# EavianWoo/SinGS

Measured on AMD Instinct MI355X. Metric: rendered views/sec fwd+bwd, 200k Gaussians @1080p, higher is better.
Workload: dtype f32; 1 GPU; S(200000,1920,1080,deg=3,seed=3): 200000 Gaussians, 1920x1080, SH deg 3, fwd+bwd, R=780064 (tile,Gaussian) pairs, every view of a step within 0.1 % of that (cameras a few cm apart), frame-parallel dp1; gaussians=200000, width=1920, height=1080, sh_degree=3, num_rendered=780064, tile_list_max=135, frames_per_launch=8, streams=2, regularisers=False, forward_only=False, hip_graph=False, reduction=fold of 2 gradient row(s) for 16 views + collective in 1 chunk(s), gradient_rows=2, parallelism=dp1

## Files before the change

sings_amd/csrc/sg_binning.hip:

```cpp
#include "sg_sort.h"
#include <atomic>

#define SG_SCAN_NQ 6
__device__ __forceinline__ void sg_scan_derive(uint32_t v, uint32_t q[SG_SCAN_NQ])
{
    const uint32_t seg = sg_nseg(v);
    q[0] = v; q[1] = seg ? seg : 1u; q[2] = seg; q[3] = v > SG_WSORT_MAX ? 1u : 0u; q[4] = sg_group_slots(v);
    q[5] = (v > SG_WSORT_MAX / 2 ? 1u : 0u) | (v > SG_TILE_ROW_LONG / 2 ? 1u << 20 : 0u);
}

__device__ __forceinline__ void sg_publish_count(unsigned long long *signal, uint32_t R, uint32_t flags)
{
    if (signal) __hip_atomic_store(signal, (1ull << 63) | ((unsigned long long)flags << 32) | R, __ATOMIC_RELEASE, __HIP_MEMORY_SCOPE_SYSTEM);
}

template <int SG_SCAN_BS>
__global__ void __launch_bounds__(SG_SCAN_BS)
sg_tile_scan_kernel(int T, int gx, int tpt, const uint32_t *__restrict__ tile_count,
                    uint2 *__restrict__ ranges, uint32_t *__restrict__ cursor, uint32_t *__restrict__ header,
                    uint32_t cap, uint32_t sort_cap, uint32_t rank_cap, uint4 *__restrict__ plan,
                    uint32_t *__restrict__ ck_start, uint32_t items_cap, int short_lists, unsigned long long *signal, size_t bin_stride,
                    int direct)
{
    constexpr int NQ = SG_SCAN_NQ;
    __shared__ uint32_t wsum[NQ][SG_SCAN_BS / 64];
    __shared__ uint32_t carry[NQ];
    {
        const size_t off = (size_t)blockIdx.y * bin_stride;
        tile_count = sg_at(tile_count, off); ranges = sg_at(ranges, off); cursor = sg_at(cursor, off); header = sg_at(header, off);
        plan = sg_at(plan, off); ck_start = sg_at(ck_start, off);
        if (signal) signal += blockIdx.y;
    }
    const int tid = threadIdx.x, lane = tid & 63, wid = tid >> 6;
    const int first = blockIdx.x * SG_SCAN_BS * tpt;
// ... 518 lines not shown
        if (tid == 0 && L.gslot > g0) atomicAdd(&header[7], L.gslot - g0);
    }
}

__global__ void __launch_bounds__(256)
sg_group_sort_kernel(const uint32_t *__restrict__ header, const uint2 *__restrict__ groups, const uint64_t *__restrict__ pair_keys,
                     const uint64_t *__restrict__ scratch, uint32_t *__restrict__ point_list, uint64_t *__restrict__ point_keys,
                     size_t bin_stride)
{
    __shared__ uint64_t s[SG_WSORT_MAX + SG_RANKSORT_MAX];
    {
        const size_t off = (size_t)blockIdx.y * bin_stride;
        header = sg_at(header, off); groups = sg_at(groups, off); pair_keys = sg_at(pair_keys, off); scratch = sg_at(scratch, off);
        point_list = sg_at(point_list, off); point_keys = sg_at(point_keys, off);
    }
    const int tid = threadIdx.x;
    const uint32_t nslots = header[1] || header[7] == 0u ? 0u : header[6];
    for (uint32_t gi = blockIdx.x; gi < nslots; gi += gridDim.x) {
        const uint2 g = groups[gi];
        const uint32_t len = g.y & 0x7ffu, tile = g.y >> 11;
        if (len == 0u) continue;
        const uint32_t start = g.x & ~SG_GROUP_IN_A;
        const uint64_t *src = ((g.x & SG_GROUP_IN_A) ? pair_keys : scratch) + start;
        __syncthreads();
        sg_sort_short_list(src, (int)len, s, s + SG_WSORT_MAX, tid);
        for (uint32_t i = tid; i < len; i += 256) {
            const uint64_t k = s[i];
            point_list[start + i] = (uint32_t)k;
            if (point_keys) point_keys[start + i] = ((uint64_t)tile << 32) | (k >> 32);
        }
    }
}

static bool sg_dyn_lds_limit(int which, const void *fn, int bytes)
{
    static std::atomic<signed char> state[2][64];
    int dev = 0;
    if (hipGetDevice(&dev) != hipSuccess || dev < 0 || dev >= 64)
        return hipFuncSetAttribute(fn, hipFuncAttributeMaxDynamicSharedMemorySize, bytes) == hipSuccess || ((void)hipGetLastError(), false);
    signed char st = state[which][dev].load(std::memory_order_acquire);
    if (st == 0) {
        st = hipFuncSetAttribute(fn, hipFuncAttributeMaxDynamicSharedMemorySize, bytes) == hipSuccess ? 1 : -1;
        if (st < 0) (void)hipGetLastError();
        state[which][dev].store(st, std::memory_order_release);
    }
    return st > 0;
}

void sg_launch_binning(const SgCam &c, const SgBatch &bt, int P, const int32_t *radii, SgGeom g, SgBin b, size_t cap,
                       int write_keys, hipStream_t st)
{
    (void)radii; (void)P;
    const unsigned K = (unsigned)bt.K;
    const int T = c.gx * c.gy;
    const uint32_t cap32 = sg_cap32(cap);
    uint64_t *pk = write_keys ? b.point_keys : (uint64_t *)nullptr;
    const int short_lists = (c.flags & SG_FLAG_SHORT_LISTS) ? 1 : 0;
    const uint32_t key_pitch = sg_key_pitch(c.gx, c.gy, c.flags);
    const int direct = key_pitch ? 1 : 0;
    bool fused = T <= SG_SS_MAX_TILES && (K == 1 || sg_lds_hist(c.gx, c.gy) || direct);
    if (fused && (size_t)T * 4 + 1024 > 64 * 1024)
        fused = sg_dyn_lds_limit(0, (const void *)sg_scan_scatter_kernel, SG_SS_MAX_TILES * 4);
    if (fused) {
        sg_prof_begin(SG_K_TILE_SCAN, st);
        size_t want = (cap + 4 * SG_SS_THREADS - 1) / (4 * SG_SS_THREADS);
        const int grid = direct ? SG_DIRECT_SCAN_WGS : (int)(want < 8 ? 8 : (want > 256 ? 256 : want));
        hipLaunchKernelGGL(sg_scan_scatter_kernel, dim3(grid, K), dim3(SG_SS_THREADS), (size_t)T * 4, st, T, c.gx, b.tile_count, b.ranges,
                           b.cursor, b.header, cap32, sg_sort_items_cap(T, cap), sg_rank_items_cap(cap), b.plan, b.ck_start,
                           sg_items_cap(T, cap), b.pair_gid, b.pair_tile, b.pair_local, g.depth, b.pair_keys, b.sort_items,
                           b.rank_items, b.items, b.item_w, short_lists, c.count_signal, bt.bin, bt.geom,
                           sg_lds_hist(c.gx, c.gy) ? b.rec_valid : (uint8_t *)nullptr, direct);
        sg_prof_end(SG_K_TILE_SCAN, st);
    } else {
        sg_prof_begin(SG_K_TILE_SCAN, st);
        const int tpt = (T + 65535) / 65536 > 0 ? (T + 65535) / 65536 : 1;
        const int sgrid = (T + 1024 * tpt - 1) / (1024 * tpt) > 0 ? (T + 1024 * tpt - 1) / (1024 * tpt) : 1;
        hipLaunchKernelGGL((sg_tile_scan_kernel<1024>), dim3(sgrid, K), dim3(1024), 0, st, T, c.gx, tpt, b.tile_count, b.ranges, b.cursor,
                           b.header, cap32, sg_sort_items_cap(T, cap), sg_rank_items_cap(cap), b.plan, b.ck_start,
                           sg_items_cap(T, cap), short_lists, c.count_signal, bt.bin, direct);
        sg_prof_end(SG_K_TILE_SCAN, st);
        sg_prof_begin(SG_K_TILE_SCATTER, st);
        size_t want = (((direct || cap < (size_t)T) ? (size_t)T : cap) + 255) / 256;
        int grid = (int)(want < 1 ? 1 : (want > 8192 ? 8192 : want));
        hipLaunchKernelGGL(sg_pair_scatter_kernel, dim3(grid, K), dim3(256), 0, st, b.header, b.pair_gid, b.pair_tile,
                           b.pair_local, g.depth, b.cursor, b.pair_keys, cap32, T, b.plan, b.sort_items, b.rank_items,
                           sg_sort_items_cap(T, cap), sg_rank_items_cap(cap), b.items, sg_items_cap(T, cap), b.item_w, bt.bin, bt.geom,
                           sg_lds_hist(c.gx, c.gy) ? b.rec_valid : (uint8_t *)nullptr, direct);
        sg_prof_end(SG_K_TILE_SCATTER, st);
    }
    if (short_lists) return;
    sg_prof_begin(SG_K_TILE_SORT, st);
    const uint32_t pgrid = sg_sort_items_cap(T, cap) < 512 ? sg_sort_items_cap(T, cap) : 512;
    uint32_t resident = SG_PT_U * SG_PT_THREADS;
    size_t dyn = (size_t)resident * 8 + (size_t)SG_PT_FINE * 4;
    if (!sg_dyn_lds_limit(1, (const void *)sg_tile_partition_kernel, (int)dyn)) { resident = SG_PT_NB; dyn = (size_t)SG_PT_NB * 8; }
    hipLaunchKernelGGL(sg_tile_partition_kernel, dim3(pgrid, K), dim3(SG_PT_THREADS), dyn, st, b.header, b.sort_items,
                       b.pair_keys, b.point_keys, b.rank_items, sg_rank_items_cap(cap), b.point_list, pk,
                       resident > SG_PT_NB ? resident : 0u, bt.bin, b.tile_keys, key_pitch);
    const uint32_t ggrid = sg_rank_items_cap(cap) < 256 ? sg_rank_items_cap(cap) : 256;
    hipLaunchKernelGGL(sg_group_sort_kernel, dim3(ggrid, K), dim3(256), 0, st, b.header, b.rank_items, b.pair_keys, b.point_keys,
                       b.point_list, pk, bt.bin);
    sg_prof_end(SG_K_TILE_SORT, st);
}
```

sings_amd/csrc/sg_host.h:

```cpp
#pragma once
#include "sg_common.h"

#include <math.h>
#include <stdarg.h>
#include <stdio.h>

static inline int sg_failf(const char *fmt, ...)
{
    char msg[256];
    va_list ap;
    va_start(ap, fmt);
    vsnprintf(msg, sizeof msg, fmt, ap);
    va_end(ap);
    return sg_set_error(msg, hipSuccess);
}

static inline int sg_launched(const char *what)
{
    const hipError_t e = hipGetLastError();
    return e == hipSuccess ? 0 : sg_set_error(what, e);
}

static inline void sg_ssim_window(float w[11])
{
    float g[11];
    double s = 0.0;
    for (int x = 0; x < 11; x++) { g[x] = (float)exp(-(double)((x - 5) * (x - 5)) / (2.0 * 1.5 * 1.5)); s += (double)g[x]; }
    for (int x = 0; x < 11; x++) w[x] = g[x] / (float)s;
}

#define SG_CHECK_LAST(what, s, st)                                           \
    do {                                                                     \
        hipError_t e_ = hipGetLastError();                                   \
        if (e_ != hipSuccess) return sg_set_error(what, e_);                 \
        if ((s)->debug) {                                                    \
            e_ = hipStreamSynchronize(st);                                   \
            if (e_ != hipSuccess) return sg_set_error(what, e_);             \
        }                                                                    \
    } while (0)

int sg_launch_linear_bwd_fan(int N, int Cin, int Cout, int act, const float *z, const float *dh, const float *W, float *dz_out,
                             float *dx_out, const SgLinearSide *side, hipStream_t st);
void sg_launch_scales_head(int N, const float *z, float *scales, float *aux, const float *dscales, const float *daux, float *dz,
                           hipStream_t st);
void sg_launch_rows_laplacian(int R, int V, int C, const float *x, const int *row_ptr, const int *col, const float *val,
                              const float *rscale, const int *t_row_ptr, const int *t_row, const float *t_val, void *ws, float *g_ws,
                              float *loss, const float *upstream, float *dL_dx, hipStream_t st);

static inline bool sg_order_applies(const SgCam &c) { return !sg_lds_hist(c.gx, c.gy) && sg_key_pitch_of(false, c.flags) != 0u; }
void sg_launch_preprocess_fwd_ordered(const SgCam &c, const SgBatch &bt, int P, const float *means3D, const float *shs,
                                      const float *colors_precomp, const float *opacities, const float *scales,
                                      const float *rotations, const float *cov3D_precomp, SgGeom g, SgBin b,
                                      size_t cap, int32_t *radii, const uint32_t *order, hipStream_t st);
// ... 2 lines not shown
```

sings_amd/csrc/sg_preprocess.hip:

```cpp
#include "sg_project.h"
#include "sg_host.h"

template <int D, bool NOBIN>
__global__ void __launch_bounds__(256)
sg_preprocess_fwd_kernel(SgCam c, SgBatch bt, int P, const float *__restrict__ means3D,
                         const float *__restrict__ shs, const float *__restrict__ colors_precomp,
                         const float *__restrict__ opacities, const float *__restrict__ scales,
                         const float *__restrict__ rotations, const float *__restrict__ cov3D_precomp,
                         SgGeom g, SgBin bn, uint32_t cap, int32_t *__restrict__ radii, int hist_tiles, int nblocks)
{
    extern __shared__ uint32_t sg_hist_lds[];
    __shared__ uint32_t scratch_all[4][NOBIN ? 1 : 256];
    int gblock, frame;
    if (!sg_block_frame((int)blockIdx.x, bt.K, nblocks, gblock, frame)) return;
    c = sg_frame(c, frame, bt.cam_stride); g = sg_frame(g, (size_t)frame * bt.geom); bn = sg_frame(bn, (size_t)frame * bt.bin);
    radii += (size_t)frame * bt.P;
    const int idx = gblock * 256 + (int)threadIdx.x;
    const int wave = threadIdx.x >> 6;
    const bool live = idx < P;
    constexpr int nc = (D + 1) * (D + 1);
    float sh[nc * 3];
    if (shs && live) {
        const float *src = shs + (size_t)idx * c.M * 3;
        if (D == 3 && c.M == 16) {
// ... 63 lines not shown
    if (P <= 0) return;
    const int nblocks = (P + 255) / 256;
    dim3 grid(sg_frame_grid(nblocks, bt.K)), block(256);
    const int ht = sg_lds_hist(c.gx, c.gy) ? (int)sg_ctr_count((uint32_t)c.gx, (uint32_t)c.gy) : 0;
    const bool ord = order && sg_order_applies(c);
#define SG_PPO(DD, OO) hipLaunchKernelGGL((sg_preprocess_fwd_kernel<DD, OO>), grid, block, (size_t)ht * 4, st, c, bt, P, means3D, shs, \
                                     colors_precomp, opacities, scales, rotations, cov3D_precomp, g, b, sg_cap32(cap), radii, ht, nblocks)
#define SG_PP(DD) do { if (ord) SG_PPO(DD, true); else SG_PPO(DD, false); } while (0)
    int D = colors_precomp ? 0 : c.D;
    sg_prof_begin(SG_K_PREPROCESS_FWD, st);
    switch (D) { case 0: SG_PP(0); break; case 1: SG_PP(1); break; case 2: SG_PP(2); break; default: SG_PP(3); break; }
    if (ord)
        hipLaunchKernelGGL(sg_bin_ordered_kernel, dim3(nblocks, bt.K), block, 0, st, bt, P, g, b, c.gx, sg_key_pitch_of(false, c.flags), order);
    sg_prof_end(SG_K_PREPROCESS_FWD, st);
#undef SG_PP
#undef SG_PPO
}

#define SG_PBWD_PARAMS SgCam c, int P, const float *__restrict__ means3D, const float *__restrict__ shs,                              \
                       const float *__restrict__ colors_precomp, const float *__restrict__ scales,                                \
                       const float *__restrict__ rotations, const float *__restrict__ cov3D_precomp,                              \
                       const int32_t *__restrict__ radii, SgGeom g, SgRec grec,                                                   \
                       size_t cap, const uint32_t *__restrict__ header, const uint8_t *__restrict__ rec_valid, float *__restrict__ dL_dmeans3D, float *__restrict__ dL_dmeans2D, \
                       float *__restrict__ dL_dsh, float *__restrict__ dL_dcolors,                                                \
                       float *__restrict__ dL_dopacity, float *__restrict__ dL_dscales,                                           \
                       float *__restrict__ dL_drots, float *__restrict__ dL_dcov3D
#define SG_PBWD_AUX 0
#include "sg_preprocess_bwd.inc"
#undef SG_PBWD_AUX
#define SG_PBWD_AUX 1
#include "sg_preprocess_bwd.inc"
#undef SG_PBWD_AUX

#define SG_GROW_VEC 4
template <int D>
__global__ void __launch_bounds__(256) __attribute__((amdgpu_waves_per_eu(4, 4)))
sg_gauss_frame_bwd_kernel(SgCam c, SgBatch bt, int P, const float *__restrict__ means3D, const float *__restrict__ shs,
                          const float *__restrict__ scales, const float *__restrict__ rotations,
                          const float *__restrict__ cov3D_precomp, const int32_t *__restrict__ radii, SgGeom g, SgRec grec,
                          size_t cap, const uint32_t *__restrict__ header, const uint8_t *__restrict__ rec_valid,
                          float4 *__restrict__ rows, float *__restrict__ dL_dmeans2D, int nblocks)
{
    __shared__ float lds_all[4][32 * SG_ROW_LDS];
    int gblock, frame;
    if (!sg_block_frame((int)blockIdx.x, bt.K, nblocks, gblock, frame)) return;
    c = sg_frame(c, frame, bt.cam_stride); g = sg_frame(g, (size_t)frame * bt.geom); grec = sg_frame(grec, (size_t)frame * bt.rec);
    header = sg_at(header, (size_t)frame * bt.bin); rec_valid = sg_at(rec_valid, (size_t)frame * bt.bin);
    radii += (size_t)frame * bt.P;
    const int idx = gblock * 256 + (int)threadIdx.x;
    const int lane = threadIdx.x & 63, wave = threadIdx.x >> 6;
    if (idx - lane >= P) return;
    const bool live = idx < P;
    const bool vis = live && radii[idx] > 0 && header[1] == 0u;
    const int Mrows = c.M;
    constexpr int nc = (D + 1) * (D + 1);
    const bool want_sh = shs != nullptr;
    float4 rc = make_float4(0, 0, 0, 0);
    float p[3] = { 0, 0, 0 }, s3[3] = { 0, 0, 0 }, q[4] = { 0, 0, 0, 0 }, sh[nc * 3];
    uint32_t flags = 0;
    if (vis) {
        { const uint2 sl = g.slot[idx]; rc.y = __uint_as_float(sl.x); rc.w = __uint_as_float(sl.y); }
        flags = g.flags[idx];
        p[0] = means3D[3 * idx]; p[1] = means3D[3 * idx + 1]; p[2] = means3D[3 * idx + 2];
        if (!cov3D_precomp) {
            s3[0] = scales[3 * idx]; s3[1] = scales[3 * idx + 1]; s3[2] = scales[3 * idx + 2];
            q[0] = rotations[4 * idx]; q[1] = rotations[4 * idx + 1]; q[2] = rotations[4 * idx + 2]; q[3] = rotations[4 * idx + 3];
        }
    }
    float a9[9];
    sg_sum_records_coop(grec, cap, vis, rc, lane, lds_all[wave], a9, rec_valid);
    if (!live) return;
    float *m2 = dL_dmeans2D + 3 * ((size_t)frame * bt.P + idx);
    if (!vis) { m2[0] = 0.0f; m2[1] = 0.0f; m2[2] = 0.0f; return; }
    SgGaussGrad G;
    sg_project_bwd<D>(c, p, s3, q, cov3D_precomp ? cov3D_precomp + 6 * (size_t)idx : nullptr, nullptr, flags, a9, false, nullptr, G);
    m2[0] = G.g2[0]; m2[1] = G.g2[1]; m2[2] = 0.0f;
    float dRGB[3] = { G.dcol[0], G.dcol[1], G.dcol[2] };
    if (want_sh) {
        int ish = idx;
        asm volatile("" : "+v"(ish), "+v"(G.dmean[2]), "+v"(G.drot[3]));
        const float *src = shs + (size_t)ish * Mrows * 3;
        if (D == 3 && Mrows == 16) {
#pragma unroll
            for (int k = 0; k < nc * 3 / 4; k++) {
                const float4 v = ((const float4 *)src)[k];
                sh[4 * k] = v.x; sh[4 * k + 1] = v.y; sh[4 * k + 2] = v.z; sh[4 * k + 3] = v.w;
            }
        } else {
#pragma unroll
            for (int k = 0; k < nc * 3; k++) sh[k] = src[k];
        }
        float dorig[3] = { p[0] - c.campos[0], p[1] - c.campos[1], p[2] - c.campos[2] };
        float sum2 = dorig[0] * dorig[0] + dorig[1] * dorig[1] + dorig[2] * dorig[2];
        float len = sqrtf(sum2);
        float dir[3] = { dorig[0] / len, dorig[1] / len, dorig[2] / len };
        float db[48];
        sg_sh_basis_grad<D>(dir, db);
#pragma unroll
        for (int ch = 0; ch < 3; ch++) dRGB[ch] = (flags >> ch) & 1u ? 0.0f : G.dcol[ch];
        float ddir[3] = { 0, 0, 0 };
#pragma unroll
        for (int k = 1; k < nc; k++)
#pragma unroll
            for (int ch = 0; ch < 3; ch++) {
                float sv = sh[3 * k + ch] * dRGB[ch];
                ddir[0] += db[3 * k] * sv; ddir[1] += db[3 * k + 1] * sv; ddir[2] += db[3 * k + 2] * sv;
            }
        float inv32 = 1.0f / sqrtf(sum2 * sum2 * sum2);
        float vx = dorig[0], vy = dorig[1], vz = dorig[2];
        G.dmean[0] += ((sum2 - vx * vx) * ddir[0] - vy * vx * ddir[1] - vz * vx * ddir[2]) * inv32;
        G.dmean[1] += (-vx * vy * ddir[0] + (sum2 - vy * vy) * ddir[1] - vz * vy * ddir[2]) * inv32;
        G.dmean[2] += (-vx * vz * ddir[0] - vy * vz * ddir[1] + (sum2 - vz * vz) * ddir[2]) * inv32;
    }
    float4 *o = rows + SG_GROW_VEC * ((size_t)frame * bt.P + idx);
    o[0] = make_float4(G.dmean[0], G.dmean[1], G.dmean[2], G.dop);
    if (cov3D_precomp) {
        o[1] = make_float4(G.g6[0], G.g6[1], G.g6[2], G.g6[3]);
        o[2] = make_float4(G.g6[4], G.g6[5], 0.0f, 0.0f);
    } else {
        o[1] = make_float4(G.dsc[0], G.dsc[1], G.dsc[2], 0.0f);
        o[2] = make_float4(G.drot[0], G.drot[1], G.drot[2], G.drot[3]);
    }
    o[3] = make_float4(dRGB[0], dRGB[1], dRGB[2], 0.0f);
}

template <int D, bool ACC>
__global__ void __launch_bounds__(256) __attribute__((amdgpu_waves_per_eu(4, 4)))
sg_gauss_sum_frames_kernel(SgCam c0, SgBatch bt, int P, const float *__restrict__ means3D, const int32_t *__restrict__ radii0,
                           const uint32_t *__restrict__ header0, const float4 *__restrict__ rows, int g6rows,
                           float *__restrict__ dL_dmeans3D, float *__restrict__ dL_dsh, float *__restrict__ dL_dcolors,
                           float *__restrict__ dL_dopacity, float *__restrict__ dL_dscales, float *__restrict__ dL_drots,
                           float *__restrict__ dL_dcov3D)
{
    __shared__ float lds_all[4][32 * SG_ROW_LDS];
    const int idx = blockIdx.x * blockDim.x + threadIdx.x;
    const int lane = threadIdx.x & 63, wave = threadIdx.x >> 6;
    const int g0 = idx - lane;
    if (g0 >= P) return;
    const bool live = idx < P;
    const int Mrows = c0.M;
    const int nframes = bt.K;
    constexpr int nc = (D + 1) * (D + 1);
    const bool want_sh = dL_dsh != nullptr;
    const bool planar = c0.flags & SG_FLAG_SH_PLANAR;
    const bool staged = D == 3 && Mrows == 16 && want_sh && !planar;
    bool vis_n = live && radii0[idx] > 0 && header0[1] == 0u;
    const float4 z4 = make_float4(0, 0, 0, 0);
    float4 n[SG_GROW_VEC] = { z4, z4, z4, z4 };
    if (vis_n) {
        const float4 *src = rows + SG_GROW_VEC * (size_t)idx;
#pragma unroll
        for (int v = 0; v < SG_GROW_VEC; v++) n[v] = src[v];
    }
    float p[3] = { 0, 0, 0 };
    if (live) { p[0] = means3D[3 * idx]; p[1] = means3D[3 * idx + 1]; p[2] = means3D[3 * idx + 2]; }
    constexpr int NA = 4 * SG_GROW_VEC - 1;
    static_assert(NA * 64 <= 32 * SG_ROW_LDS, "the geometry sums fit the wave's staging block");
    float *sA = lds_all[wave] + lane;
    float A[NA];
#pragma unroll
    for (int k = 0; k < NA; k++) A[k] = 0.0f;
    float acc[nc * 3];
#pragma unroll
    for (int k = 0; k < nc * 3; k++) acc[k] = 0.0f;
    if (ACC && live) {
#pragma unroll
        for (int k = 0; k < 3; k++) A[k] = dL_dmeans3D[3 * idx + k];
        A[3] = dL_dopacity[idx];
        if (g6rows) {
#pragma unroll
            for (int k = 0; k < 6; k++) A[4 + k] = dL_dcov3D ? dL_dcov3D[6 * idx + k] : 0.0f;
        } else {
#pragma unroll
            for (int k = 0; k < 3; k++) A[4 + k] = dL_dscales ? dL_dscales[3 * idx + k] : 0.0f;
#pragma unroll
            for (int k = 0; k < 4; k++) A[8 + k] = dL_drots ? dL_drots[4 * idx + k] : 0.0f;
        }
#pragma unroll
        for (int k = 0; k < 3; k++) A[12 + k] = dL_dcolors ? dL_dcolors[3 * idx + k] : 0.0f;
        if (want_sh) {
            const float *row = dL_dsh + (size_t)idx * Mrows * 3;
#pragma unroll
            for (int k = 0; k < nc * 3; k++) acc[k] = planar ? dL_dsh[((size_t)(k / 3) * P + idx) * 3 + k % 3] : row[k];
        }
    }
#pragma unroll
    for (int k = 0; k < NA; k++) sA[64 * k] = A[k];
#pragma unroll 1
    for (int f = 0; f < nframes; f++) {
        const bool vis = vis_n;
        const bool first = !ACC && f == 0;
        int ln = lane;
        asm volatile("" : "+v"(ln));
        float *sAf = lds_all[wave] + ln;
#pragma unroll
        for (int v = 0; v < SG_GROW_VEC; v++) {
            const float r[4] = { n[v].x, n[v].y, n[v].z, n[v].w };
#pragma unroll
            for (int k = 0; k < 4; k++)
                if (4 * v + k < NA) sAf[64 * (4 * v + k)] = first ? r[k] : r[k] + sAf[64 * (4 * v + k)];
        }
        const float dRGB[3] = { n[3].x, n[3].y, n[3].z };
        if (f + 1 < nframes) {
            vis_n = live && radii0[(size_t)(f + 1) * bt.P + idx] > 0 && sg_at(header0, (size_t)(f + 1) * bt.bin)[1] == 0u;
#pragma unroll
            for (int v = 0; v < SG_GROW_VEC; v++) n[v] = z4;
            if (vis_n) {
                const float4 *src = rows + SG_GROW_VEC * ((size_t)(f + 1) * bt.P + idx);
#pragma unroll
                for (int v = 0; v < SG_GROW_VEC; v++) n[v] = src[v];
            }
        }
        if (want_sh && vis) {
            const float *campos = c0.campos + 3 * (size_t)f * (size_t)bt.cam_stride;
            float dorig[3] = { p[0] - campos[0], p[1] - campos[1], p[2] - campos[2] };
            float sum2 = dorig[0] * dorig[0] + dorig[1] * dorig[1] + dorig[2] * dorig[2];
            float len = sqrtf(sum2);
            float dir[3] = { dorig[0] / len, dorig[1] / len, dorig[2] / len };
            float bas[16];
            sg_sh_basis<D>(dir, bas);
#pragma unroll
            for (int k = 0; k < nc; k++)
#pragma unroll
                for (int ch = 0; ch < 3; ch++)
                    acc[3 * k + ch] = first ? bas[k] * dRGB[ch] : acc[3 * k + ch] + bas[k] * dRGB[ch];
        }
    }
#pragma unroll
    for (int k = 0; k < NA; k++) A[k] = sA[64 * k];
    __builtin_amdgcn_s_waitcnt(0xC07F);
    __builtin_amdgcn_wave_barrier();
    if (want_sh && planar) {
        if (live) {
#pragma unroll
            for (int k = 0; k < nc * 3; k++) dL_dsh[((size_t)(k / 3) * P + idx) * 3 + k % 3] = acc[k];
        }
    } else if (want_sh) {
        if (staged) {
            float *L = lds_all[wave];
#pragma unroll
            for (int h = 0; h < 2; h++) {
                if ((lane >> 5) == h) {
#pragma unroll
                    for (int k = 0; k < nc * 3 / 4; k++)
                        *(float4 *)(L + (lane & 31) * SG_ROW_LDS + 4 * k) = make_float4(acc[4 * k], acc[4 * k + 1], acc[4 * k + 2], acc[4 * k + 3]);
                }
                __builtin_amdgcn_s_waitcnt(0xC07F);
                __builtin_amdgcn_wave_barrier();
                sg_rows48_store(dL_dsh, g0 + 32 * h, P, lane, L, 32, false);
                __builtin_amdgcn_s_waitcnt(0xC07F);
                __builtin_amdgcn_wave_barrier();
            }
        } else if (live) {
            float *dsh_row = dL_dsh + (size_t)idx * Mrows * 3;
#pragma unroll
            for (int k = 0; k < nc * 3; k++) dsh_row[k] = acc[k];
            if (!ACC)
                for (int k = nc * 3; k < Mrows * 3; k++) dsh_row[k] = 0.0f;
        }
    }
    if (!live) return;
    dL_dmeans3D[3 * idx] = A[0]; dL_dmeans3D[3 * idx + 1] = A[1]; dL_dmeans3D[3 * idx + 2] = A[2];
    dL_dopacity[idx] = A[3];
    if (dL_dcolors) { dL_dcolors[3 * idx] = A[12]; dL_dcolors[3 * idx + 1] = A[13]; dL_dcolors[3 * idx + 2] = A[14]; }
    if (g6rows) {
        if (dL_dcov3D) {
#pragma unroll
            for (int k = 0; k < 6; k++) dL_dcov3D[6 * idx + k] = A[4 + k];
        }
    } else {
        if (dL_dscales) { dL_dscales[3 * idx] = A[4]; dL_dscales[3 * idx + 1] = A[5]; dL_dscales[3 * idx + 2] = A[6]; }
        if (dL_drots) { dL_drots[4 * idx] = A[8]; dL_drots[4 * idx + 1] = A[9]; dL_drots[4 * idx + 2] = A[10]; dL_drots[4 * idx + 3] = A[11]; }
    }
}

void sg_launch_preprocess_bwd(const SgCam &c, const SgBatch &bt, int P, const float *means3D, const float *shs,
                              const float *colors_precomp, const float *opacities, const float *scales,
                              const float *rotations, const float *cov3D_precomp,
                              const int32_t *radii, SgGeom g, SgRec grec, size_t cap, const uint32_t *header, const uint8_t *rec_valid,
                              float4 *a9buf, float *dL_dmeans3D, float *dL_dmeans2D, float *dL_dsh,
                              float *dL_dcolors, float *dL_dopacity, float *dL_dscales,
                              float *dL_drots, float *dL_dcov3D, int accumulate, hipStream_t st, const float *dz)
{
    (void)opacities;
    if (P <= 0) return;
    const int nblocks = (P + 255) / 256;
    dim3 grid(nblocks), block(256);
    int D = shs ? c.D : 0;
    if (bt.K > 1 && ((shs && dL_dcolors) || (!cov3D_precomp && dL_dcov3D))) {
        SgBatch one = bt;
        one.K = 1;
        for (int f = 0; f < bt.K; f++)
            sg_launch_preprocess_bwd(sg_frame(c, f, bt.cam_stride), one, P, means3D, shs, colors_precomp, opacities, scales, rotations,
                                     cov3D_precomp, radii + (size_t)f * bt.P, sg_frame(g, (size_t)f * bt.geom),
                                     sg_frame(grec, (size_t)f * bt.rec), cap, sg_at(header, (size_t)f * bt.bin),
                                     sg_at(rec_valid, (size_t)f * bt.bin), nullptr, dL_dmeans3D, dL_dmeans2D + 3 * (size_t)f * bt.P,
                                     dL_dsh, dL_dcolors, dL_dopacity, dL_dscales, dL_drots, dL_dcov3D, accumulate || f > 0, st, nullptr);
        return;
    }
#define SG_PB1(DD, AA) hipLaunchKernelGGL((sg_preprocess_bwd_kernel<DD, AA>), grid, block, 0, st, c, P, means3D, shs, \
                                     colors_precomp, scales, rotations, cov3D_precomp, radii, g,            \
                                     grec, cap, header, rec_valid, dL_dmeans3D, dL_dmeans2D, dL_dsh, dL_dcolors, \
                                     dL_dopacity, dL_dscales, dL_drots, dL_dcov3D)
#define SG_PBK(DD, AA) do {                                                                                                        \
        hipLaunchKernelGGL((sg_gauss_frame_bwd_kernel<DD>), dim3(sg_frame_grid(nblocks, bt.K)), block, 0, st, c, bt, P, means3D,   \
                           shs, scales, rotations, cov3D_precomp, radii, g, grec, cap, header, rec_valid, a9buf, dL_dmeans2D,      \
                           nblocks);                                                                                               \
        hipLaunchKernelGGL((sg_gauss_sum_frames_kernel<DD, AA>), grid, block, 0, st, c, bt, P, means3D, radii, header, a9buf,      \
                           cov3D_precomp != nullptr, dL_dmeans3D, dL_dsh, dL_dcolors, dL_dopacity, dL_dscales, dL_drots,           \
                           dL_dcov3D);                                                                                             \
    } while (0)
#define SG_PB2(DD, AA) do { if (bt.K == 1) SG_PB1(DD, AA); else SG_PBK(DD, AA); } while (0)
#define SG_PB(DD) do { if (accumulate) SG_PB2(DD, true); else SG_PB2(DD, false); } while (0)
    sg_prof_begin(SG_K_PREPROCESS_BWD, st);
#define SG_PBA(DD) hipLaunchKernelGGL((sg_preprocess_bwd_aux_kernel<DD>), grid, block, 0, st, c, P, means3D, shs,            \
                                     colors_precomp, scales, rotations, cov3D_precomp, radii, g,            \
                                     grec, cap, header, rec_valid, dL_dmeans3D, dL_dmeans2D, dL_dsh, dL_dcolors, \
                                     dL_dopacity, dL_dscales, dL_drots, dL_dcov3D, dz)
    if (dz)
        switch (D) { case 0: SG_PBA(0); break; case 1: SG_PBA(1); break; case 2: SG_PBA(2); break; default: SG_PBA(3); break; }
    else
    switch (D) { case 0: SG_PB(0); break; case 1: SG_PB(1); break; case 2: SG_PB(2); break; default: SG_PB(3); break; }
#undef SG_PBA
    sg_prof_end(SG_K_PREPROCESS_BWD, st);
#undef SG_PB
#undef SG_PB2
#undef SG_PB1
#undef SG_PBK
}
```

Measured before the change: 5621 views/s.

## Fuse per-frame Gaussian backward and cross-frame gradient sum into one LDS kernel

Replaces the two-kernel multi-frame preprocess backward (per-frame rows written to a global buffer, then a summing kernel) with one kernel. Each block covers 64 Gaussians, with one wave per frame. The waves write their gradient rows and SH basis into LDS, then all threads reduce across frames and write the final gradients. This removes the global round-trip of the per-frame row buffer and one launch. In exchange it needs up to K×8KB of dynamic LDS and a K×64-thread block, which may limit occupancy. The LDS-attribute helper is moved into a shared header so it can be reused.

```diff
diff --git a/sings_amd/csrc/sg_binning.hip b/sings_amd/csrc/sg_binning.hip
--- a/sings_amd/csrc/sg_binning.hip
+++ b/sings_amd/csrc/sg_binning.hip
@@ -1,5 +1,5 @@
 #include "sg_sort.h"
-#include <atomic>
+#include "sg_host.h"
 
 #define SG_SCAN_NQ 6
 __device__ __forceinline__ void sg_scan_derive(uint32_t v, uint32_t q[SG_SCAN_NQ])
@@ -584,20 +584,7 @@
     }
 }
 
-static bool sg_dyn_lds_limit(int which, const void *fn, int bytes)
-{
-    static std::atomic<signed char> state[2][64];
-    int dev = 0;
-    if (hipGetDevice(&dev) != hipSuccess || dev < 0 || dev >= 64)
-        return hipFuncSetAttribute(fn, hipFuncAttributeMaxDynamicSharedMemorySize, bytes) == hipSuccess || ((void)hipGetLastError(), false);
-    signed char st = state[which][dev].load(std::memory_order_acquire);
-    if (st == 0) {
-        st = hipFuncSetAttribute(fn, hipFuncAttributeMaxDynamicSharedMemorySize, bytes) == hipSuccess ? 1 : -1;
-        if (st < 0) (void)hipGetLastError();
-        state[which][dev].store(st, std::memory_order_release);
-    }
-    return st > 0;
-}
+static SgLdsLimit sg_ss_lds_limit, sg_pt_lds_limit;
 
 void sg_launch_binning(const SgCam &c, const SgBatch &bt, int P, const int32_t *radii, SgGeom g, SgBin b, size_t cap,
                        int write_keys, hipStream_t st)
@@ -612,7 +599,7 @@
     const int direct = key_pitch ? 1 : 0;
     bool fused = T <= SG_SS_MAX_TILES && (K == 1 || sg_lds_hist(c.gx, c.gy) || direct);
     if (fused && (size_t)T * 4 + 1024 > 64 * 1024)
-        fused = sg_dyn_lds_limit(0, (const void *)sg_scan_scatter_kernel, SG_SS_MAX_TILES * 4);
+        fused = sg_dyn_lds_limit(sg_ss_lds_limit, (const void *)sg_scan_scatter_kernel, SG_SS_MAX_TILES * 4);
     if (fused) {
         sg_prof_begin(SG_K_TILE_SCAN, st);
         size_t want = (cap + 4 * SG_SS_THREADS - 1) / (4 * SG_SS_THREADS);
@@ -645,7 +632,7 @@
     const uint32_t pgrid = sg_sort_items_cap(T, cap) < 512 ? sg_sort_items_cap(T, cap) : 512;
     uint32_t resident = SG_PT_U * SG_PT_THREADS;
     size_t dyn = (size_t)resident * 8 + (size_t)SG_PT_FINE * 4;
-    if (!sg_dyn_lds_limit(1, (const void *)sg_tile_partition_kernel, (int)dyn)) { resident = SG_PT_NB; dyn = (size_t)SG_PT_NB * 8; }
+    if (!sg_dyn_lds_limit(sg_pt_lds_limit, (const void *)sg_tile_partition_kernel, (int)dyn)) { resident = SG_PT_NB; dyn = (size_t)SG_PT_NB * 8; }
     hipLaunchKernelGGL(sg_tile_partition_kernel, dim3(pgrid, K), dim3(SG_PT_THREADS), dyn, st, b.header, b.sort_items,
                        b.pair_keys, b.point_keys, b.rank_items, sg_rank_items_cap(cap), b.point_list, pk,
                        resident > SG_PT_NB ? resident : 0u, bt.bin, b.tile_keys, key_pitch);
diff --git a/sings_amd/csrc/sg_host.h b/sings_amd/csrc/sg_host.h
--- a/sings_amd/csrc/sg_host.h
+++ b/sings_amd/csrc/sg_host.h
@@ -1,6 +1,7 @@
 #pragma once
 #include "sg_common.h"
 
+#include <atomic>
 #include <math.h>
 #include <stdarg.h>
 #include <stdio.h>
@@ -19,6 +20,21 @@
 {
     const hipError_t e = hipGetLastError();
     return e == hipSuccess ? 0 : sg_set_error(what, e);
+}
+
+struct SgLdsLimit { std::atomic<signed char> state[64]; };
+static inline bool sg_dyn_lds_limit(SgLdsLimit &m, const void *fn, int bytes)
+{
+    int dev = 0;
+    if (hipGetDevice(&dev) != hipSuccess || dev < 0 || dev >= 64)
+        return hipFuncSetAttribute(fn, hipFuncAttributeMaxDynamicSharedMemorySize, bytes) == hipSuccess || ((void)hipGetLastError(), false);
+    signed char st = m.state[dev].load(std::memory_order_acquire);
+    if (st == 0) {
+        st = hipFuncSetAttribute(fn, hipFuncAttributeMaxDynamicSharedMemorySize, bytes) == hipSuccess ? 1 : -1;
+        if (st < 0) (void)hipGetLastError();
+        m.state[dev].store(st, std::memory_order_release);
+    }
+    return st > 0;
 }
 
 static inline void sg_ssim_window(float w[11])
diff --git a/sings_amd/csrc/sg_preprocess.hip b/sings_amd/csrc/sg_preprocess.hip
--- a/sings_amd/csrc/sg_preprocess.hip
+++ b/sings_amd/csrc/sg_preprocess.hip
@@ -119,246 +119,208 @@
 #include "sg_preprocess_bwd.inc"
 #undef SG_PBWD_AUX
 
-#define SG_GROW_VEC 4
-template <int D>
-__global__ void __launch_bounds__(256) __attribute__((amdgpu_waves_per_eu(4, 4)))
-sg_gauss_frame_bwd_kernel(SgCam c, SgBatch bt, int P, const float *__restrict__ means3D, const float *__restrict__ shs,
-                          const float *__restrict__ scales, const float *__restrict__ rotations,
-                          const float *__restrict__ cov3D_precomp, const int32_t *__restrict__ radii, SgGeom g, SgRec grec,
-                          size_t cap, const uint32_t *__restrict__ header, const uint8_t *__restrict__ rec_valid,
-                          float4 *__restrict__ rows, float *__restrict__ dL_dmeans2D, int nblocks)
-{
-    __shared__ float lds_all[4][32 * SG_ROW_LDS];
-    int gblock, frame;
-    if (!sg_block_frame((int)blockIdx.x, bt.K, nblocks, gblock, frame)) return;
-    c = sg_frame(c, frame, bt.cam_stride); g = sg_frame(g, (size_t)frame * bt.geom); grec = sg_frame(grec, (size_t)frame * bt.rec);
-    header = sg_at(header, (size_t)frame * bt.bin); rec_valid = sg_at(rec_valid, (size_t)frame * bt.bin);
-    radii += (size_t)frame * bt.P;
-    const int idx = gblock * 256 + (int)threadIdx.x;
-    const int lane = threadIdx.x & 63, wave = threadIdx.x >> 6;
-    if (idx - lane >= P) return;
-    const bool live = idx < P;
-    const bool vis = live && radii[idx] > 0 && header[1] == 0u;
-    const int Mrows = c.M;
+#define SG_GF_PITCH 31
+#define SG_GF_BLOCK 2048
+#define SG_GF_RGB 11
+#define SG_GF_BAS 14
+#define SG_GF_VIS 30
+#define SG_GF_BATCH 8
+static_assert(64 * SG_GF_PITCH <= SG_GF_BLOCK && SG_REC_CHUNK * 12 <= SG_GF_BLOCK, "a wave's LDS block holds its rows and a record chunk");
+template <int D, bool ACC>
+__global__ void __launch_bounds__(1024)
+sg_gauss_frames_bwd_kernel(SgCam c, SgBatch bt, int P, const float *__restrict__ means3D, const float *__restrict__ shs,
+                           const float *__restrict__ scales, const float *__restrict__ rotations,
+                           const float *__restrict__ cov3D_precomp, const int32_t *__restrict__ radii, SgGeom g, SgRec grec,
+                           size_t cap, const uint32_t *__restrict__ header, const uint8_t *__restrict__ rec_valid,
+                           float *__restrict__ dL_dmeans2D, float *__restrict__ dL_dmeans3D, float *__restrict__ dL_dsh,
+                           float *__restrict__ dL_dcolors, float *__restrict__ dL_dopacity, float *__restrict__ dL_dscales,
+                           float *__restrict__ dL_drots, float *__restrict__ dL_dcov3D)
+{
+    extern __shared__ float sg_gf_lds[];
+    const int lane = threadIdx.x & 63;
+    const int frame = __builtin_amdgcn_readfirstlane((int)(threadIdx.x >> 6));
+    const int g0 = (int)blockIdx.x * 64;
     constexpr int nc = (D + 1) * (D + 1);
     const bool want_sh = shs != nullptr;
-    float4 rc = make_float4(0, 0, 0, 0);
-    float p[3] = { 0, 0, 0 }, s3[3] = { 0, 0, 0 }, q[4] = { 0, 0, 0, 0 }, sh[nc * 3];
-    uint32_t flags = 0;
-    if (vis) {
-        { const uint2 sl = g.slot[idx]; rc.y = __uint_as_float(sl.x); rc.w = __uint_as_float(sl.y); }
-        flags = g.flags[idx];
-        p[0] = means3D[3 * idx]; p[1] = means3D[3 * idx + 1]; p[2] = means3D[3 * idx + 2];
-        if (!cov3D_precomp) {
-            s3[0] = scales[3 * idx]; s3[1] = scales[3 * idx + 1]; s3[2] = scales[3 * idx + 2];
-            q[0] = rotations[4 * idx]; q[1] = rotations[4 * idx + 1]; q[2] = rotations[4 * idx + 2]; q[3] = rotations[4 * idx + 3];
-        }
-    }
-    float a9[9];
-    sg_sum_records_coop(grec, cap, vis, rc, lane, lds_all[wave], a9, rec_valid);
-    if (!live) return;
-    float *m2 = dL_dmeans2D + 3 * ((size_t)frame * bt.P + idx);
-    if (!vis) { m2[0] = 0.0f; m2[1] = 0.0f; m2[2] = 0.0f; return; }
-    SgGaussGrad G;
-    sg_project_bwd<D>(c, p, s3, q, cov3D_precomp ? cov3D_precomp + 6 * (size_t)idx : nullptr, nullptr, flags, a9, false, nullptr, G);
-    m2[0] = G.g2[0]; m2[1] = G.g2[1]; m2[2] = 0.0f;
-    float dRGB[3] = { G.dcol[0], G.dcol[1], G.dcol[2] };
+    {
+        const int idx = g0 + lane;
+        float *L = sg_gf_lds + frame * SG_GF_BLOCK;
+        const SgCam cf = sg_frame(c, frame, bt.cam_stride);
+        const SgGeom gf = sg_frame(g, (size_t)frame * bt.geom);
+        const SgRec grf = sg_frame(grec, (size_t)frame * bt.rec);
+        const uint32_t *hf = sg_at(header, (size_t)frame * bt.bin);
+        const uint8_t *rvf = sg_at(rec_valid, (size_t)frame * bt.bin);
+        const int32_t *rad = radii + (size_t)frame * bt.P;
+        const bool live = idx < P;
+        const bool vis = live && rad[idx] > 0 && hf[1] == 0u;
+        const int Mrows = cf.M;
+        float4 rc = make_float4(0, 0, 0, 0);
+        float p[3] = { 0, 0, 0 }, s3[3] = { 0, 0, 0 }, q[4] = { 0, 0, 0, 0 }, sh[nc * 3];
+        uint32_t flags = 0;
+        if (vis) {
+            { const uint2 sl = gf.slot[idx]; rc.y = __uint_as_float(sl.x); rc.w = __uint_as_float(sl.y); }
+            flags = gf.flags[idx];
+            p[0] = means3D[3 * idx]; p[1] = means3D[3 * idx + 1]; p[2] = means3D[3 * idx + 2];
+            if (!cov3D_precomp) {
+                s3[0] = scales[3 * idx]; s3[1] = scales[3 * idx + 1]; s3[2] = scales[3 * idx + 2];
+                q[0] = rotations[4 * idx]; q[1] = rotations[4 * idx + 1]; q[2] = rotations[4 * idx + 2]; q[3] = rotations[4 * idx + 3];
+            }
+        }
+        float a9[9];
+        sg_sum_records_coop(grf, cap, vis, rc, lane, L, a9, rvf);
+        float *row = L + lane * SG_GF_PITCH;
+        row[SG_GF_VIS] = vis ? 1.0f : 0.0f;
+        if (!vis) {
+#pragma unroll
+            for (int k = 0; k < SG_GF_BAS; k++) row[k] = 0.0f;
+        }
+        if (live) {
+            float *m2 = dL_dmeans2D + 3 * ((size_t)frame * bt.P + idx);
+            if (!vis) { m2[0] = 0.0f; m2[1] = 0.0f; m2[2] = 0.0f; }
+        }
+        if (vis) {
+            float *m2 = dL_dmeans2D + 3 * ((size_t)frame * bt.P + idx);
+            SgGaussGrad G;
+            sg_project_bwd<D>(cf, p, s3, q, cov3D_precomp ? cov3D_precomp + 6 * (size_t)idx : nullptr, nullptr, flags, a9, false, nullptr, G);
+            m2[0] = G.g2[0]; m2[1] = G.g2[1]; m2[2] = 0.0f;
+            float dRGB[3] = { G.dcol[0], G.dcol[1], G.dcol[2] };
+            if (want_sh) {
+                int ish = idx;
+                asm volatile("" : "+v"(ish), "+v"(G.dmean[2]), "+v"(G.drot[3]));
+                const float *src = shs + (size_t)ish * Mrows * 3;
+                if (D == 3 && Mrows == 16) {
+#pragma unroll
+                    for (int k = 0; k < nc * 3 / 4; k++) {
+                        const float4 v = ((const float4 *)src)[k];
+                        sh[4 * k] = v.x; sh[4 * k + 1] = v.y; sh[4 * k + 2] = v.z; sh[4 * k + 3] = v.w;
+                    }
+                } else {
+#pragma unroll
+                    for (int k = 0; k < nc * 3; k++) sh[k] = src[k];
+                }
+                float dorig[3] = { p[0] - cf.campos[0], p[1] - cf.campos[1], p[2] - cf.campos[2] };
+                float sum2 = dorig[0] * dorig[0] + dorig[1] * dorig[1] + dorig[2] * dorig[2];
+                float len = sqrtf(sum2);
+                float dir[3] = { dorig[0] / len, dorig[1] / len, dorig[2] / len };
+                {
+                    float bas[16];
+                    sg_sh_basis<D>(dir, bas);
+#pragma unroll
+                    for (int k = 0; k < nc; k++) row[SG_GF_BAS + k] = bas[k];
+                }
+                float db[48];
+                sg_sh_basis_grad<D>(dir, db);
+#pragma unroll
+                for (int ch = 0; ch < 3; ch++) dRGB[ch] = (flags >> ch) & 1u ? 0.0f : G.dcol[ch];
+                float ddir[3] = { 0, 0, 0 };
+#pragma unroll
+                for (int k = 1; k < nc; k++)
+#pragma unroll
+                    for (int ch = 0; ch < 3; ch++) {
+                        float sv = sh[3 * k + ch] * dRGB[ch];
+                        ddir[0] += db[3 * k] * sv; ddir[1] += db[3 * k + 1] * sv; ddir[2] += db[3 * k + 2] * sv;
+                    }
+                float inv32 = 1.0f / sqrtf(sum2 * sum2 * sum2);
+                float vx = dorig[0], vy = dorig[1], vz = dorig[2];
+                G.dmean[0] += ((sum2 - vx * vx) * ddir[0] - vy * vx * ddir[1] - vz * vx * ddir[2]) * inv32;
+                G.dmean[1] += (-vx * vy * ddir[0] + (sum2 - vy * vy) * ddir[1] - vz * vy * ddir[2]) * inv32;
+                G.dmean[2] += (-vx * vz * ddir[0] - vy * vz * ddir[1] + (sum2 - vz * vz) * ddir[2]) * inv32;
+            }
+            row[0] = G.dmean[0]; row[1] = G.dmean[1]; row[2] = G.dmean[2]; row[3] = G.dop;
+            if (cov3D_precomp) {
+#pragma unroll
+                for (int k = 0; k < 6; k++) row[4 + k] = G.g6[k];
+            } else {
+                row[4] = G.dsc[0]; row[5] = G.dsc[1]; row[6] = G.dsc[2];
+                row[7] = G.drot[0]; row[8] = G.drot[1]; row[9] = G.drot[2]; row[10] = G.drot[3];
+            }
+            row[SG_GF_RGB] = dRGB[0]; row[SG_GF_RGB + 1] = dRGB[1]; row[SG_GF_RGB + 2] = dRGB[2];
+        }
+    }
+    __syncthreads();
+    const int tid = (int)threadIdx.x, nthr = bt.K * 64, nframes = bt.K;
+    const int nlive = P - g0 < 64 ? P - g0 : 64;
     if (want_sh) {
-        int ish = idx;
-        asm volatile("" : "+v"(ish), "+v"(G.dmean[2]), "+v"(G.drot[3]));
-        const float *src = shs + (size_t)ish * Mrows * 3;
-        if (D == 3 && Mrows == 16) {
-#pragma unroll
-            for (int k = 0; k < nc * 3 / 4; k++) {
-                const float4 v = ((const float4 *)src)[k];
-                sh[4 * k] = v.x; sh[4 * k + 1] = v.y; sh[4 * k + 2] = v.z; sh[4 * k + 3] = v.w;
-            }
-        } else {
-#pragma unroll
-            for (int k = 0; k < nc * 3; k++) sh[k] = src[k];
-        }
-        float dorig[3] = { p[0] - c.campos[0], p[1] - c.campos[1], p[2] - c.campos[2] };
-        float sum2 = dorig[0] * dorig[0] + dorig[1] * dorig[1] + dorig[2] * dorig[2];
-        float len = sqrtf(sum2);
-        float dir[3] = { dorig[0] / len, dorig[1] / len, dorig[2] / len };
-        float db[48];
-        sg_sh_basis_grad<D>(dir, db);
-#pragma unroll
-        for (int ch = 0; ch < 3; ch++) dRGB[ch] = (flags >> ch) & 1u ? 0.0f : G.dcol[ch];
-        float ddir[3] = { 0, 0, 0 };
-#pragma unroll
-        for (int k = 1; k < nc; k++)
-#pragma unroll
-            for (int ch = 0; ch < 3; ch++) {
-                float sv = sh[3 * k + ch] * dRGB[ch];
-                ddir[0] += db[3 * k] * sv; ddir[1] += db[3 * k + 1] * sv; ddir[2] += db[3 * k + 2] * sv;
-            }
-        float inv32 = 1.0f / sqrtf(sum2 * sum2 * sum2);
-        float vx = dorig[0], vy = dorig[1], vz = dorig[2];
-        G.dmean[0] += ((sum2 - vx * vx) * ddir[0] - vy * vx * ddir[1] - vz * vx * ddir[2]) * inv32;
-        G.dmean[1] += (-vx * vy * ddir[0] + (sum2 - vy * vy) * ddir[1] - vz * vy * ddir[2]) * inv32;
-        G.dmean[2] += (-vx * vz * ddir[0] - vy * vz * ddir[1] + (sum2 - vz * vz) * ddir[2]) * inv32;
-    }
-    float4 *o = rows + SG_GROW_VEC * ((size_t)frame * bt.P + idx);
-    o[0] = make_float4(G.dmean[0], G.dmean[1], G.dmean[2], G.dop);
-    if (cov3D_precomp) {
-        o[1] = make_float4(G.g6[0], G.g6[1], G.g6[2], G.g6[3]);
-        o[2] = make_float4(G.g6[4], G.g6[5], 0.0f, 0.0f);
-    } else {
-        o[1] = make_float4(G.dsc[0], G.dsc[1], G.dsc[2], 0.0f);
-        o[2] = make_float4(G.drot[0], G.drot[1], G.drot[2], G.drot[3]);
-    }
-    o[3] = make_float4(dRGB[0], dRGB[1], dRGB[2], 0.0f);
-}
-
-template <int D, bool ACC>
-__global__ void __launch_bounds__(256) __attribute__((amdgpu_waves_per_eu(4, 4)))
-sg_gauss_sum_frames_kernel(SgCam c0, SgBatch bt, int P, const float *__restrict__ means3D, const int32_t *__restrict__ radii0,
-                           const uint32_t *__restrict__ header0, const float4 *__restrict__ rows, int g6rows,
-                           float *__restrict__ dL_dmeans3D, float *__restrict__ dL_dsh, float *__restrict__ dL_dcolors,
-                           float *__restrict__ dL_dopacity, float *__restrict__ dL_dscales, float *__restrict__ dL_drots,
-                           float *__restrict__ dL_dcov3D)
-{
-    __shared__ float lds_all[4][32 * SG_ROW_LDS];
-    const int idx = blockIdx.x * blockDim.x + threadIdx.x;
-    const int lane = threadIdx.x & 63, wave = threadIdx.x >> 6;
-    const int g0 = idx - lane;
-    if (g0 >= P) return;
-    const bool live = idx < P;
-    const int Mrows = c0.M;
-    const int nframes = bt.K;
-    constexpr int nc = (D + 1) * (D + 1);
-    const bool want_sh = dL_dsh != nullptr;
-    const bool planar = c0.flags & SG_FLAG_SH_PLANAR;
-    const bool staged = D == 3 && Mrows == 16 && want_sh && !planar;
-    bool vis_n = live && radii0[idx] > 0 && header0[1] == 0u;
-    const float4 z4 = make_float4(0, 0, 0, 0);
-    float4 n[SG_GROW_VEC] = { z4, z4, z4, z4 };
-    if (vis_n) {
-        const float4 *src = rows + SG_GROW_VEC * (size_t)idx;
-#pragma unroll
-        for (int v = 0; v < SG_GROW_VEC; v++) n[v] = src[v];
-    }
-    float p[3] = { 0, 0, 0 };
-    if (live) { p[0] = means3D[3 * idx]; p[1] = means3D[3 * idx + 1]; p[2] = means3D[3 * idx + 2]; }
-    constexpr int NA = 4 * SG_GROW_VEC - 1;
-    static_assert(NA * 64 <= 32 * SG_ROW_LDS, "the geometry sums fit the wave's staging block");
-    float *sA = lds_all[wave] + lane;
-    float A[NA];
-#pragma unroll
-    for (int k = 0; k < NA; k++) A[k] = 0.0f;
-    float acc[nc * 3];
-#pragma unroll
-    for (int k = 0; k < nc * 3; k++) acc[k] = 0.0f;
-    if (ACC && live) {
-#pragma unroll
-        for (int k = 0; k < 3; k++) A[k] = dL_dmeans3D[3 * idx + k];
-        A[3] = dL_dopacity[idx];
-        if (g6rows) {
-#pragma unroll
-            for (int k = 0; k < 6; k++) A[4 + k] = dL_dcov3D ? dL_dcov3D[6 * idx + k] : 0.0f;
-        } else {
-#pragma unroll
-            for (int k = 0; k < 3; k++) A[4 + k] = dL_dscales ? dL_dscales[3 * idx + k] : 0.0f;
-#pragma unroll
-            for (int k = 0; k < 4; k++) A[8 + k] = dL_drots ? dL_drots[4 * idx + k] : 0.0f;
-        }
-#pragma unroll
-        for (int k = 0; k < 3; k++) A[12 + k] = dL_dcolors ? dL_dcolors[3 * idx + k] : 0.0f;
-        if (want_sh) {
-            const float *row = dL_dsh + (size_t)idx * Mrows * 3;
-#pragma unroll
-            for (int k = 0; k < nc * 3; k++) acc[k] = planar ? dL_dsh[((size_t)(k / 3) * P + idx) * 3 + k % 3] : row[k];
-        }
-    }
-#pragma unroll
-    for (int k = 0; k < NA; k++) sA[64 * k] = A[k];
-#pragma unroll 1
-    for (int f = 0; f < nframes; f++) {
-        const bool vis = vis_n;
-        const bool first = !ACC && f == 0;
-        int ln = lane;
-        asm volatile("" : "+v"(ln));
-        float *sAf = lds_all[wave] + ln;
-#pragma unroll
-        for (int v = 0; v < SG_GROW_VEC; v++) {
-            const float r[4] = { n[v].x, n[v].y, n[v].z, n[v].w };
-#pragma unroll
-            for (int k = 0; k < 4; k++)
-                if (4 * v + k < NA) sAf[64 * (4 * v + k)] = first ? r[k] : r[k] + sAf[64 * (4 * v + k)];
-        }
-        const float dRGB[3] = { n[3].x, n[3].y, n[3].z };
-        if (f + 1 < nframes) {
-            vis_n = live && radii0[(size_t)(f + 1) * bt.P + idx] > 0 && sg_at(header0, (size_t)(f + 1) * bt.bin)[1] == 0u;
-#pragma unroll
-            for (int v = 0; v < SG_GROW_VEC; v++) n[v] = z4;
-            if (vis_n) {
-                const float4 *src = rows + SG_GROW_VEC * ((size_t)(f + 1) * bt.P + idx);
-#pragma unroll
-                for (int v = 0; v < SG_GROW_VEC; v++) n[v] = src[v];
-            }
-        }
-        if (want_sh && vis) {
-            const float *campos = c0.campos + 3 * (size_t)f * (size_t)bt.cam_stride;
-            float dorig[3] = { p[0] - campos[0], p[1] - campos[1], p[2] - campos[2] };
-            float sum2 = dorig[0] * dorig[0] + dorig[1] * dorig[1] + dorig[2] * dorig[2];
-            float len = sqrtf(sum2);
-            float dir[3] = { dorig[0] / len, dorig[1] / len, dorig[2] / len };
-            float bas[16];
-            sg_sh_basis<D>(dir, bas);
-#pragma unroll
-            for (int k = 0; k < nc; k++)
-#pragma unroll
-                for (int ch = 0; ch < 3; ch++)
-                    acc[3 * k + ch] = first ? bas[k] * dRGB[ch] : acc[3 * k + ch] + bas[k] * dRGB[ch];
-        }
-    }
-#pragma unroll
-    for (int k = 0; k < NA; k++) A[k] = sA[64 * k];
-    __builtin_amdgcn_s_waitcnt(0xC07F);
-    __builtin_amdgcn_wave_barrier();
-    if (want_sh && planar) {
-        if (live) {
-#pragma unroll
-            for (int k = 0; k < nc * 3; k++) dL_dsh[((size_t)(k / 3) * P + idx) * 3 + k % 3] = acc[k];
-        }
-    } else if (want_sh) {
-        if (staged) {
-            float *L = lds_all[wave];
-#pragma unroll
-            for (int h = 0; h < 2; h++) {
-                if ((lane >> 5) == h) {
-#pragma unroll
-                    for (int k = 0; k < nc * 3 / 4; k++)
-                        *(float4 *)(L + (lane & 31) * SG_ROW_LDS + 4 * k) = make_float4(acc[4 * k], acc[4 * k + 1], acc[4 * k + 2], acc[4 * k + 3]);
+        const bool planar = c.flags & SG_FLAG_SH_PLANAR;
+        const int Mrows = c.M;
+        const int nitems = 64 * (planar ? nc : Mrows);
+        for (int it = tid; it < nitems; it += nthr) {
+            int j, k;
+            float *dst;
+            if (planar) { k = it >> 6; j = it & 63; dst = dL_dsh + ((size_t)k * P + (size_t)(g0 + j)) * 3; }
+            else { j = it / Mrows; k = it - j * Mrows; dst = dL_dsh + ((size_t)(g0 + j) * Mrows + k) * 3; }
+            if (j >= nlive) continue;
+            if (k >= nc) {
+                if (!ACC) { dst[0] = 0.0f; dst[1] = 0.0f; dst[2] = 0.0f; }
+                continue;
+            }
+            float a0 = 0.0f, a1 = 0.0f, a2 = 0.0f;
+            if (ACC) { a0 = dst[0]; a1 = dst[1]; a2 = dst[2]; }
+            const float *r = sg_gf_lds + j * SG_GF_PITCH;
+            for (int f0 = 0; f0 < nframes; f0 += SG_GF_BATCH) {
+                float vv[SG_GF_BATCH], bb[SG_GF_BATCH], d0[SG_GF_BATCH], d1[SG_GF_BATCH], d2[SG_GF_BATCH];
+#pragma unroll
+                for (int u = 0; u < SG_GF_BATCH; u++) {
+                    const float *rf = r + (f0 + u < nframes ? f0 + u : nframes - 1) * SG_GF_BLOCK;
+                    vv[u] = rf[SG_GF_VIS]; bb[u] = rf[SG_GF_BAS + k];
+                    d0[u] = rf[SG_GF_RGB]; d1[u] = rf[SG_GF_RGB + 1]; d2[u] = rf[SG_GF_RGB + 2];
                 }
-                __builtin_amdgcn_s_waitcnt(0xC07F);
-                __builtin_amdgcn_wave_barrier();
-                sg_rows48_store(dL_dsh, g0 + 32 * h, P, lane, L, 32, false);
-                __builtin_amdgcn_s_waitcnt(0xC07F);
-                __builtin_amdgcn_wave_barrier();
-            }
-        } else if (live) {
-            float *dsh_row = dL_dsh + (size_t)idx * Mrows * 3;
-#pragma unroll
-            for (int k = 0; k < nc * 3; k++) dsh_row[k] = acc[k];
-            if (!ACC)
-                for (int k = nc * 3; k < Mrows * 3; k++) dsh_row[k] = 0.0f;
-        }
-    }
-    if (!live) return;
-    dL_dmeans3D[3 * idx] = A[0]; dL_dmeans3D[3 * idx + 1] = A[1]; dL_dmeans3D[3 * idx + 2] = A[2];
-    dL_dopacity[idx] = A[3];
-    if (dL_dcolors) { dL_dcolors[3 * idx] = A[12]; dL_dcolors[3 * idx + 1] = A[13]; dL_dcolors[3 * idx + 2] = A[14]; }
-    if (g6rows) {
-        if (dL_dcov3D) {
-#pragma unroll
-            for (int k = 0; k < 6; k++) dL_dcov3D[6 * idx + k] = A[4 + k];
-        }
-    } else {
-        if (dL_dscales) { dL_dscales[3 * idx] = A[4]; dL_dscales[3 * idx + 1] = A[5]; dL_dscales[3 * idx + 2] = A[6]; }
-        if (dL_drots) { dL_drots[4 * idx] = A[8]; dL_drots[4 * idx + 1] = A[9]; dL_drots[4 * idx + 2] = A[10]; dL_drots[4 * idx + 3] = A[11]; }
-    }
+#pragma unroll
+                for (int u = 0; u < SG_GF_BATCH; u++) asm volatile("" : "+v"(vv[u]), "+v"(bb[u]), "+v"(d0[u]), "+v"(d1[u]), "+v"(d2[u]));
+#pragma unroll
+                for (int u = 0; u < SG_GF_BATCH; u++) {
+                    const bool seen = f0 + u < nframes && vv[u] != 0.0f, first = !ACC && f0 + u == 0;
+                    const float p0 = bb[u] * d0[u], p1 = bb[u] * d1[u], p2 = bb[u] * d2[u];
+                    a0 = seen ? (first ? p0 : a0 + p0) : a0;
+                    a1 = seen ? (first ? p1 : a1 + p1) : a1;
+                    a2 = seen ? (first ? p2 : a2 + p2) : a2;
+                }
+            }
+            dst[0] = a0; dst[1] = a1; dst[2] = a2;
+        }
+    }
+    const bool g6rows = cov3D_precomp != nullptr;
+    const int nB = g6rows ? 6 * 64 : 3 * 64, nC = g6rows ? 0 : 4 * 64;
+    const int ngeo = 3 * 64 + 64 + nB + nC + (dL_dcolors ? 3 * 64 : 0);
+    for (int it = tid; it < ngeo; it += nthr) {
+        int t = it, j, s;
+        float *dst;
+        if (t < 3 * 64) { j = t / 3; s = t - 3 * j; dst = dL_dmeans3D + 3 * (size_t)g0 + t; }
+        else if ((t -= 3 * 64) < 64) { j = t; s = 3; dst = dL_dopacity + (size_t)g0 + t; }
+        else if ((t -= 64) < nB) {
+            if (g6rows) { j = t / 6; s = 4 + t - 6 * j; dst = dL_dcov3D ? dL_dcov3D + 6 * (size_t)g0 + t : nullptr; }
+            else { j = t / 3; s = 4 + t - 3 * j; dst = dL_dscales ? dL_dscales + 3 * (size_t)g0 + t : nullptr; }
+        }
+        else if ((t -= nB) < nC) { j = t >> 2; s = 7 + (t & 3); dst = dL_drots ? dL_drots + 4 * (size_t)g0 + t : nullptr; }
+        else { t -= nC; j = t / 3; s = SG_GF_RGB + t - 3 * j; dst = dL_dcolors + 3 * (size_t)g0 + t; }
+        if (!dst || j >= nlive) continue;
+        float a = 0.0f;
+        if (ACC) a = *dst;
+        const float *r = sg_gf_lds + j * SG_GF_PITCH;
+        for (int f0 = 0; f0 < nframes; f0 += SG_GF_BATCH) {
+            float v[SG_GF_BATCH];
+#pragma unroll
+            for (int u = 0; u < SG_GF_BATCH; u++) v[u] = r[(f0 + u < nframes ? f0 + u : nframes - 1) * SG_GF_BLOCK + s];
+#pragma unroll
+            for (int u = 0; u < SG_GF_BATCH; u++) asm volatile("" : "+v"(v[u]));
+#pragma unroll
+            for (int u = 0; u < SG_GF_BATCH; u++)
+                if (f0 + u < nframes) a = (!ACC && f0 + u == 0) ? v[u] : v[u] + a;
+        }
+        *dst = a;
+    }
+}
+template <int D, bool ACC> static bool sg_gauss_frames_lds(size_t bytes)
+{
+    static SgLdsLimit limit;
+    return bytes <= 64 * 1024 ||
+           sg_dyn_lds_limit(limit, (const void *)sg_gauss_frames_bwd_kernel<D, ACC>, SG_MAX_FRAMES * SG_GF_BLOCK * 4);
+}
+static bool sg_gauss_frames_fit(int D, bool acc, size_t bytes)
+{
+#define SG_GF_FIT(DD) (acc ? sg_gauss_frames_lds<DD, true>(bytes) : sg_gauss_frames_lds<DD, false>(bytes))
+    switch (D) { case 0: return SG_GF_FIT(0); case 1: return SG_GF_FIT(1); case 2: return SG_GF_FIT(2); default: return SG_GF_FIT(3); }
+#undef SG_GF_FIT
 }
 
 void sg_launch_preprocess_bwd(const SgCam &c, const SgBatch &bt, int P, const float *means3D, const float *shs,
@@ -369,12 +331,13 @@
                               float *dL_dcolors, float *dL_dopacity, float *dL_dscales,
                               float *dL_drots, float *dL_dcov3D, int accumulate, hipStream_t st, const float *dz)
 {
-    (void)opacities;
+    (void)opacities; (void)a9buf;
     if (P <= 0) return;
     const int nblocks = (P + 255) / 256;
     dim3 grid(nblocks), block(256);
     int D = shs ? c.D : 0;
-    if (bt.K > 1 && ((shs && dL_dcolors) || (!cov3D_precomp && dL_dcov3D))) {
+    const size_t lds = (size_t)bt.K * SG_GF_BLOCK * sizeof(float);
+    if (bt.K > 1 && ((shs && dL_dcolors) || (!cov3D_precomp && dL_dcov3D) || !sg_gauss_frames_fit(D, accumulate != 0, lds))) {
         SgBatch one = bt;
         one.K = 1;
         for (int f = 0; f < bt.K; f++)
@@ -389,14 +352,9 @@
                                      colors_precomp, scales, rotations, cov3D_precomp, radii, g,            \
                                      grec, cap, header, rec_valid, dL_dmeans3D, dL_dmeans2D, dL_dsh, dL_dcolors, \
                                      dL_dopacity, dL_dscales, dL_drots, dL_dcov3D)
-#define SG_PBK(DD, AA) do {                                                                                                        \
-        hipLaunchKernelGGL((sg_gauss_frame_bwd_kernel<DD>), dim3(sg_frame_grid(nblocks, bt.K)), block, 0, st, c, bt, P, means3D,   \
-                           shs, scales, rotations, cov3D_precomp, radii, g, grec, cap, header, rec_valid, a9buf, dL_dmeans2D,      \
-                           nblocks);                                                                                               \
-        hipLaunchKernelGGL((sg_gauss_sum_frames_kernel<DD, AA>), grid, block, 0, st, c, bt, P, means3D, radii, header, a9buf,      \
-                           cov3D_precomp != nullptr, dL_dmeans3D, dL_dsh, dL_dcolors, dL_dopacity, dL_dscales, dL_drots,           \
-                           dL_dcov3D);                                                                                             \
-    } while (0)
+#define SG_PBK(DD, AA) hipLaunchKernelGGL((sg_gauss_frames_bwd_kernel<DD, AA>), dim3((P + 63) / 64), dim3(64 * bt.K), lds, st, c, bt, P,  \
+                                     means3D, shs, scales, rotations, cov3D_precomp, radii, g, grec, cap, header, rec_valid,          \
+                                     dL_dmeans2D, dL_dmeans3D, dL_dsh, dL_dcolors, dL_dopacity, dL_dscales, dL_drots, dL_dcov3D)
 #define SG_PB2(DD, AA) do { if (bt.K == 1) SG_PB1(DD, AA); else SG_PBK(DD, AA); } while (0)
 #define SG_PB(DD) do { if (accumulate) SG_PB2(DD, true); else SG_PB2(DD, false); } while (0)
     sg_prof_begin(SG_K_PREPROCESS_BWD, st);
```

After: 5700 views/s, median of 6. 1.4% higher.
